# rafaelvp-db/databricks-distributed-deep-learning

Hardware: AMD Instinct MI355X
Metric: ResNet-50 images/sec (whole node) (higher is better)
Workload: dtype bf16

## Files before the change

csrc/kernels/norm.hip:

```cpp
#include "ddl_common.h"
#include <cstdlib>
#include <mutex>
#include <unordered_map>

namespace {

constexpr int BN_NT = 256;

template <typename T>
__global__ __launch_bounds__(BN_NT) void bn_stats_partial_k(const T* __restrict__ x, long M, int C,
                                                            int rows_per_blk, float* __restrict__ part) {
    __shared__ float s_red[2 * BN_NT * 8];
    const int tpr = C / 8;
    const int rpi = BN_NT / tpr;
    const int tid = threadIdx.x;
    const int cg = tid % tpr, rr = tid / tpr;
    const long r0 = (long)blockIdx.x * rows_per_blk;
    const long r1 = min(M, r0 + rows_per_blk);
    float s[8], q[8];
#pragma unroll
    for (int j = 0; j < 8; ++j) { s[j] = 0.f; q[j] = 0.f; }
    long r = r0 + rr;
    for (; r + 3 * rpi < r1; r += 4 * rpi) {
        float v[4][8];
// ... 352 lines not shown
                                                           const T* __restrict__ x, const float* __restrict__ mean,
                                                           const float* __restrict__ invstd,
                                                           const float* __restrict__ coef, T* __restrict__ dx,
                                                           T* __restrict__ dres, long M, int C) {
    const int tpr = C / 8, rpb = 256 / tpr;
    const int cg = threadIdx.x % tpr, rr = threadIdx.x / tpr;
    float A[8], B[8], D[8];
    {
        float mu[8], is[8], k1[8], mb[8], mg[8];
        load8(mean + cg * 8, mu);
        load8(invstd + cg * 8, is);
        load8(coef + cg * 8, k1);
        load8(coef + C + cg * 8, mb);
        load8(coef + 2 * C + cg * 8, mg);
#pragma unroll
        for (int j = 0; j < 8; ++j) {
            A[j] = k1[j];
            B[j] = -k1[j] * is[j] * mg[j];
            D[j] = k1[j] * (mu[j] * is[j] * mg[j] - mb[j]);
        }
    }
    const long rs = (long)gridDim.x * rpb;
    auto one = [&](const float* g, const float* xv, uint32_t bits, long row) {
        float o[8], dz[8];
#pragma unroll
        for (int j = 0; j < 8; ++j) {
            dz[j] = ((bits >> j) & 1u) ? g[j] : 0.f;
            o[j] = A[j] * dz[j] + B[j] * xv[j] + D[j];
        }
        store8(dx + row * C + cg * 8, o);
        if (DRES) store8(dres + row * C + cg * 8, dz);
    };
    long r = (long)blockIdx.x * rpb + rr;
    for (; r + 3 * rs < M; r += 4 * rs) {
        float g[4][8], xv[4][8];
        uint32_t bits[4];
#pragma unroll
        for (int u = 0; u < 4; ++u) {
            load8_nt(dy + (r + u * rs) * C + cg * 8, g[u]);
            load8_nt(x + (r + u * rs) * C + cg * 8, xv[u]);
            bits[u] = RELU ? mask[(r + u * rs) * tpr + cg] : 0xffu;
        }
#pragma unroll
        for (int u = 0; u < 4; ++u) one(g[u], xv[u], bits[u], r + u * rs);
    }
    for (; r < M; r += rs) {
        float g[8], xv[8];
        load8(dy + r * C + cg * 8, g);
        load8(x + r * C + cg * 8, xv);
        one(g, xv, RELU ? mask[r * tpr + cg] : 0xffu, r);
    }
}

template <typename T> struct Raw4;
template <> struct Raw4<bf16_t> { typedef uint2 type; };
template <> struct Raw4<float> { typedef float4 type; };
__device__ __forceinline__ uint2 ld_raw4(const bf16_t* p) { return *reinterpret_cast<const uint2*>(p); }
__device__ __forceinline__ float4 ld_raw4(const float* p) { return *reinterpret_cast<const float4*>(p); }
__device__ __forceinline__ void cvt_raw4(const uint2& u, float* v) {
    v[0] = __uint_as_float(u.x << 16); v[1] = __uint_as_float(u.x & 0xffff0000u);
    v[2] = __uint_as_float(u.y << 16); v[3] = __uint_as_float(u.y & 0xffff0000u);
}
__device__ __forceinline__ void cvt_raw4(const float4& a, float* v) { v[0] = a.x; v[1] = a.y; v[2] = a.z; v[3] = a.w; }

struct Drop {
    uint64_t seed;
    uint32_t thresh;
    float scale;
    void* dres;
};
__device__ __forceinline__ uint32_t drop_bits4(const Drop& d, long idx) {
    return keep_bits4(d.seed, (uint64_t)idx, d.thresh);
}
__device__ __forceinline__ void apply4(const Drop& d, uint32_t bits, float* v) {
#pragma unroll
    for (int j = 0; j < 4; ++j) v[j] = ((bits >> j) & 1u) ? v[j] * d.scale : 0.f;
}
__device__ __forceinline__ void drop4(const Drop& d, long idx, float* v) { apply4(d, drop_bits4(d, idx), v); }

template <typename T, int VPL>
__global__ __launch_bounds__(256) void ln_fwd_k(const T* __restrict__ x, const T* __restrict__ res, long res_rows,
                                                const T* __restrict__ gamma, const T* __restrict__ beta, T* __restrict__ y,
                                                float* __restrict__ save_mean, float* __restrict__ save_rstd, long rows,
                                                int H, float eps, Drop drop) {
    const int lane = threadIdx.x & 63;
    const long row = (long)blockIdx.x * 4 + (threadIdx.x >> 6);
    if (row >= rows) return;
    float v[VPL][4];
    float s = 0.f;
#pragma unroll
    for (int k = 0; k < VPL; ++k) {
        const int col = 256 * k + 4 * lane;
        load4(x + row * H + col, v[k]);
        if (drop.thresh) drop4(drop, row * H + col, v[k]);
        if (res) {
            float r[4];
            load4(res + (row % res_rows) * H + col, r);
#pragma unroll
            for (int j = 0; j < 4; ++j) v[k][j] += r[j];
        }
#pragma unroll
        for (int j = 0; j < 4; ++j) s += v[k][j];
    }
    const float mean = wave_sum_dpp(s) / H;
    float q = 0.f;
#pragma unroll
// ... 584 lines not shown
                                                                  eps, scale, shift);
    else
        bn_eval_coeffs_k<float><<<(C + 255) / 256, 256, 0, st>>>(C, (const float*)gamma, (const float*)beta, rm, rv,
                                                                 eps, scale, shift);
    DDL_RETURN_LAUNCH();
}

template <typename T>
static void bn_apply_dispatch(const T* x, const T* res, const float* sc, const float* sh, T* y, uint8_t* mask, long n,
                              int C, int relu, hipStream_t st) {
    if (rows_ok(C) && n % C == 0) {
        const long M = n / C;
        auto k = res ? (relu ? bn_apply_rows_k<T, true, true> : bn_apply_rows_k<T, true, false>)
                     : (relu ? bn_apply_rows_k<T, false, true> : bn_apply_rows_k<T, false, false>);
        hipLaunchKernelGGL(k, dim3(rows_grid(M, C, (const void*)k)), dim3(256), 0, st, x, res, sc, sh, y, mask, M, C);
        return;
    }
    const long n8 = n / 8;
    const int g = grid_for(n8, 256, 8192);
    if (res) {
        if (relu) bn_apply_k<T, true, true><<<g, 256, 0, st>>>(x, res, sc, sh, y, mask, n8, C);
        else bn_apply_k<T, true, false><<<g, 256, 0, st>>>(x, res, sc, sh, y, mask, n8, C);
    } else {
        if (relu) bn_apply_k<T, false, true><<<g, 256, 0, st>>>(x, res, sc, sh, y, mask, n8, C);
        else bn_apply_k<T, false, false><<<g, 256, 0, st>>>(x, res, sc, sh, y, mask, n8, C);
    }
}

DDL_API int ddl_bn_apply2(int dtype, const void* x, const void* x2, const float* scale, const float* shift,
                          const float* scale2, const float* shift2, void* y, long n, int C, int relu, void* mask,
                          hipStream_t st) {
    if (n % 8 || !rows_ok(C) || n % C) return -1;
    const long M = n / C;
    uint8_t* mk = (uint8_t*)mask;
#define BA2(T) do { auto k = relu ? bn_apply2_rows_k<T, true> : bn_apply2_rows_k<T, false>; \
                    hipLaunchKernelGGL(k, dim3(rows_grid(M, C, (const void*)k)), dim3(256), 0, st, (const T*)x, (const T*)x2, \
                                       scale, shift, scale2, shift2, (T*)y, mk, M, C); } while (0)
    if (dtype == 1) BA2(bf16_t);
    else BA2(float);
#undef BA2
    DDL_RETURN_LAUNCH();
}

DDL_API int ddl_bn_apply(int dtype, const void* x, const void* res, const float* scale, const float* shift, void* y,
                         long n, int C, int relu, void* mask, hipStream_t st) {
    if (n % 8 || C % 8) return -1;
    uint8_t* mk = (uint8_t*)mask;
    if (dtype == 1) bn_apply_dispatch((const bf16_t*)x, (const bf16_t*)res, scale, shift, (bf16_t*)y, mk, n, C, relu, st);
    else bn_apply_dispatch((const float*)x, (const float*)res, scale, shift, (float*)y, mk, n, C, relu, st);
    DDL_RETURN_LAUNCH();
}

template <typename T>
static void bwd_finalize(const float* part, int nblk, float* ws, int C, long M, const T* gamma, const float* invstd,
                         T* dgamma, T* dbeta, float* coef, int acc, hipStream_t st) {
    if (merged_finalize(nblk, C)) {
        const int S = fin_slices(nblk);
        int* tk = S > 1 ? fin_tickets() : nullptr;
        if (S == 1 || tk) {
            if (!ws) ws = const_cast<float*>(part) + (long)nblk * 2 * C;
            bn_bwd_finalize2_k<T><<<dim3((C + 63) / 64, S), 1024, 0, st>>>(part, nblk, fin_rps(nblk), C, M, ws, tk,
                                                                           gamma, invstd, dgamma, dbeta, coef, acc);
            return;
        }
    }
    int nrows = nblk;
    const float* fin = collapse_partials(part, nrows, 2 * C, st, ws);
    bn_bwd_finalize_k<T><<<(C + 63) / 64, 1024, 0, st>>>(fin, nrows, C, M, gamma, invstd, dgamma, dbeta, coef, acc);
}

template <typename T>
static void bn_bwd_dispatch(const T* dy, const uint8_t* yout, const T* x, const float* mean, const float* invstd,
                            const T* gamma, long M, int C, int relu, float* part, T* dgamma, T* dbeta, float* coef,
                            T* dx, T* dres, int acc, hipStream_t st) {
    const int nblk = ddl_bn_bwd_nblk(M, C);
    const int rpi = BN_NT / (C / 8);
    long rpb = (M + nblk - 1) / nblk;
    rpb = (rpb + rpi - 1) / rpi * rpi;
    if (relu) bn_bwd_partial_k<T, true><<<nblk, BN_NT, 0, st>>>(dy, yout, x, mean, invstd, M, C, (int)rpb, part);
    else bn_bwd_partial_k<T, false><<<nblk, BN_NT, 0, st>>>(dy, yout, x, mean, invstd, M, C, (int)rpb, part);
    bwd_finalize<T>(part, nblk, nullptr, C, M, gamma, invstd, dgamma, dbeta, coef, acc, st);
    if (rows_ok(C)) {
        auto k = relu ? (dres ? bn_bwd_apply_rows_k<T, true, true> : bn_bwd_apply_rows_k<T, true, false>)
                      : (dres ? bn_bwd_apply_rows_k<T, false, true> : bn_bwd_apply_rows_k<T, false, false>);
        hipLaunchKernelGGL(k, dim3(rows_grid(M, C, (const void*)k)), dim3(256), 0, st, dy, yout, x, mean, invstd, coef,
                           dx, dres, M, C);
        return;
    }
    const long n8 = M * C / 8;
    const int g = grid_for(n8, 256, 8192);
    if (relu) {
        if (dres) bn_bwd_apply_k<T, true, true><<<g, 256, 0, st>>>(dy, yout, x, mean, invstd, coef, dx, dres, n8, C);
        else bn_bwd_apply_k<T, true, false><<<g, 256, 0, st>>>(dy, yout, x, mean, invstd, coef, dx, dres, n8, C);
    } else {
        if (dres) bn_bwd_apply_k<T, false, true><<<g, 256, 0, st>>>(dy, yout, x, mean, invstd, coef, dx, dres, n8, C);
        else bn_bwd_apply_k<T, false, false><<<g, 256, 0, st>>>(dy, yout, x, mean, invstd, coef, dx, dres, n8, C);
    }
}

DDL_API int ddl_bn_bwd(int dtype, const void* dy, const void* mask, const void* x, const float* mean,
                       const float* invstd, const void* gamma, long M, int C, int relu, float* part, void* dgamma,
                       void* dbeta, float* coef, void* dx, void* dres, int acc_params, hipStream_t st) {
    if (C % 8 || (BN_NT % (C / 8) != 0) || (relu && !mask)) return -1;
    const uint8_t* yout = (const uint8_t*)mask;
    if (dtype == 1)
        bn_bwd_dispatch((const bf16_t*)dy, yout, (const bf16_t*)x, mean, invstd, (const bf16_t*)gamma, M,
                        C, relu, part, (bf16_t*)dgamma, (bf16_t*)dbeta, coef, (bf16_t*)dx, (bf16_t*)dres, acc_params, st);
    else
        bn_bwd_dispatch((const float*)dy, yout, (const float*)x, mean, invstd, (const float*)gamma, M, C,
                        relu, part, (float*)dgamma, (float*)dbeta, coef, (float*)dx, (float*)dres, acc_params, st);
    DDL_RETURN_LAUNCH();
}

namespace {
template <typename T>
__device__ __forceinline__ void pool_grad8(const T* __restrict__ dy, const uint8_t* __restrict__ idx, long n, int h,
                                           int w, int cg, int C, int P, int Q, float* acc) {
#pragma unroll
    for (int j = 0; j < 8; ++j) acc[j] = 0.f;
    const int p_lo = h >> 1, p_hi = min(P - 1, (h + 1) >> 1);
    const int q_lo = w >> 1, q_hi = min(Q - 1, (w + 1) >> 1);
    for (int p = p_lo; p <= p_hi; ++p) {
        const int r = h - 2 * p + 1;
        for (int q = q_lo; q <= q_hi; ++q) {
            const int s_ = w - 2 * q + 1;
            const long o = ((n * P + p) * Q + q) * C + cg * 8;
            float g[8];
            load8(dy + o, g);
            const uint2 packed = *reinterpret_cast<const uint2*>(idx + o);
            const uint32_t want = (uint32_t)(r * 3 + s_);
#pragma unroll
            for (int j = 0; j < 8; ++j) {
                const uint32_t word = j < 4 ? packed.x : packed.y;
                acc[j] += ((word >> (8 * (j & 3))) & 0xffu) == want ? g[j] : 0.f;
// ... 270 lines not shown
    __shared__ float red[1024];
    const int c = blockIdx.x * 64 + (threadIdx.x & 63);
    const float s = colsum64(part, nrows, width, c, c < n, red);
    if (threadIdx.x < 64 && c < n) sink[c] = from_f<TP>(s + (acc ? to_f(sink[c]) : 0.f));
}
}

DDL_API int ddl_rows_sum_sink(int dtype, const float* part, int nblk, int width, int n, void* sink, int acc,
                              float* ws, hipStream_t st) {
    if (n > width) return -1;
    int nrows = nblk;
    const float* src = collapse_partials(part, nrows, width, st, ws);
    if (dtype == 1) rows_sum_sink_k<bf16_t><<<(n + 63) / 64, 1024, 0, st>>>(src, nrows, width, n, (bf16_t*)sink, acc);
    else rows_sum_sink_k<float><<<(n + 63) / 64, 1024, 0, st>>>(src, nrows, width, n, (float*)sink, acc);
    DDL_RETURN_LAUNCH();
}

DDL_API int ddl_bn_rows_sum(const float* part, int nblk, int width, float* out, float* ws, hipStream_t st) {
    int nrows = nblk;
    const float* src = collapse_partials(part, nrows, width, st, ws);
    rows_sum_k<<<(width + 63) / 64, 1024, 0, st>>>(src, nrows, width, out);
    DDL_RETURN_LAUNCH();
}

DDL_API int ddl_bn_stats_partials(int dtype, const void* x, long M, int C, float* part, hipStream_t st) {
    if (C % 8 || (BN_NT % (C / 8) != 0)) return -1;
    const int nblk = ddl_bn_stats_nblk(M, C);
    const int rpi = BN_NT / (C / 8);
    long rpb = (M + nblk - 1) / nblk;
    rpb = (rpb + rpi - 1) / rpi * rpi;
    if (dtype == 1) bn_stats_partial_k<bf16_t><<<nblk, BN_NT, 0, st>>>((const bf16_t*)x, M, C, (int)rpb, part);
    else bn_stats_partial_k<float><<<nblk, BN_NT, 0, st>>>((const float*)x, M, C, (int)rpb, part);
    DDL_RETURN_LAUNCH();
}

DDL_API int ddl_bn_bwd_partials(int dtype, const void* dy, const void* mask, const void* x, const float* mean,
                                const float* invstd, long M, int C, int relu, float* part, hipStream_t st) {
    if (C % 8 || (BN_NT % (C / 8) != 0) || (relu && !mask)) return -1;
    const int nblk = ddl_bn_bwd_nblk(M, C);
    const int rpi = BN_NT / (C / 8);
    long rpb = (M + nblk - 1) / nblk;
    rpb = (rpb + rpi - 1) / rpi * rpi;
    const uint8_t* mk = (const uint8_t*)mask;
#define BWP(T) do { if (relu) bn_bwd_partial_k<T, true><<<nblk, BN_NT, 0, st>>>((const T*)dy, mk, (const T*)x, mean, invstd, M, C, (int)rpb, part); \
                    else bn_bwd_partial_k<T, false><<<nblk, BN_NT, 0, st>>>((const T*)dy, mk, (const T*)x, mean, invstd, M, C, (int)rpb, part); } while (0)
    if (dtype == 1) BWP(bf16_t);
    else BWP(float);
#undef BWP
    DDL_RETURN_LAUNCH();
}

template <typename T>
static void bn_bwd_apply_only(const T* dy, const uint8_t* mk, const T* x, const float* mean, const float* invstd,
                              long M, int C, int relu, const float* coef, T* dx, T* dres, hipStream_t st) {
    if (!rows_ok(C)) return;
    auto k = relu ? (dres ? bn_bwd_apply_rows_k<T, true, true> : bn_bwd_apply_rows_k<T, true, false>)
                  : (dres ? bn_bwd_apply_rows_k<T, false, true> : bn_bwd_apply_rows_k<T, false, false>);
    hipLaunchKernelGGL(k, dim3(rows_grid(M, C, (const void*)k)), dim3(256), 0, st, dy, mk, x, mean, invstd, coef, dx,
                       dres, M, C);
}

template <typename T>
static void bn_bwd_finish_t(const T* dy, const uint8_t* mk, const T* x, const float* mean, const float* invstd,
                            const T* gamma, long M, long M_total, int C, int relu, const float* row, int nrows,
                            T* dgamma, T* dbeta, float* coef, T* dx, T* dres, int acc, hipStream_t st,
                            const float* prow = nullptr) {
    bn_bwd_finalize_k<T><<<(C + 63) / 64, 1024, 0, st>>>(row, nrows, C, M_total, gamma, invstd, dgamma, dbeta, coef,
                                                         acc, prow);
    bn_bwd_apply_only(dy, mk, x, mean, invstd, M, C, relu, coef, dx, dres, st);
}

DDL_API int ddl_bn_bwd_finish(int dtype, const void* dy, const void* mask, const void* x, const float* mean,
                              const float* invstd, const void* gamma, long M, long M_total, int C, int relu,
                              const float* row, const float* local_row, void* dgamma, void* dbeta, float* coef,
                              void* dx, void* dres, int acc_params, hipStream_t st) {
    if (!rows_ok(C) || (relu && !mask)) return -1;
    const uint8_t* mk = (const uint8_t*)mask;
    if (dtype == 1)
        bn_bwd_finish_t((const bf16_t*)dy, mk, (const bf16_t*)x, mean, invstd, (const bf16_t*)gamma, M, M_total, C,
                        relu, row, 1, (bf16_t*)dgamma, (bf16_t*)dbeta, coef, (bf16_t*)dx, (bf16_t*)dres, acc_params, st,
                        local_row);
    else
        bn_bwd_finish_t((const float*)dy, mk, (const float*)x, mean, invstd, (const float*)gamma, M, M_total, C,
                        relu, row, 1, (float*)dgamma, (float*)dbeta, coef, (float*)dx, (float*)dres, acc_params, st,
                        local_row);
    DDL_RETURN_LAUNCH();
}

DDL_API int ddl_bn_bwd_from_partials(int dtype, const float* part, int nrows, float* ws, long ws_elems,
                                     const void* dz, const void* x, const float* mean, const float* invstd,
                                     const void* gamma, long M, int C, void* dgamma, void* dbeta, float* coef, void* dx,
                                     void* dres, int acc_params, hipStream_t st) {
    if (!rows_ok(C) || dtype != 1) return -1;
    if (merged_finalize(nrows, C) && (fin_slices(nrows) == 1 || (ws && ws_elems >= (long)fin_slices(nrows) * 2 * C))) {
        bwd_finalize<bf16_t>(part, nrows, fin_slices(nrows) == 1 ? nullptr : ws, C, M, (const bf16_t*)gamma, invstd,
                             (bf16_t*)dgamma, (bf16_t*)dbeta, coef, acc_params, st);
        bn_bwd_apply_only((const bf16_t*)dz, nullptr, (const bf16_t*)x, mean, invstd, M, C, 0, coef, (bf16_t*)dx,
                          (bf16_t*)dres, st);
        DDL_RETURN_LAUNCH();
    }
    const long need = ddl_bn_partials_ws(nrows, C);
    if (need > 0 && (!ws || ws_elems < need)) return -2;
    if (need > 0) {
        bwd_finalize<bf16_t>(part, nrows, ws, C, M, (const bf16_t*)gamma, invstd, (bf16_t*)dgamma, (bf16_t*)dbeta, coef,
                             acc_params, st);
        bn_bwd_apply_only((const bf16_t*)dz, nullptr, (const bf16_t*)x, mean, invstd, M, C, 0, coef, (bf16_t*)dx,
                          (bf16_t*)dres, st);
        DDL_RETURN_LAUNCH();
    }
    bn_bwd_finish_t((const bf16_t*)dz, nullptr, (const bf16_t*)x, mean, invstd, (const bf16_t*)gamma, M, M, C, 0, part,
                    nrows, (bf16_t*)dgamma, (bf16_t*)dbeta, coef, (bf16_t*)dx, (bf16_t*)dres, acc_params, st);
    DDL_RETURN_LAUNCH();
}
```

databricks_distributed_deep_learning_amd/ops/_lib.py:

```python
from __future__ import annotations

import ctypes
import os
from typing import Optional

import torch

_PKG_DIR = os.path.dirname(os.path.dirname(os.path.abspath(__file__)))
LIB_PATH = os.environ.get("DDL_NATIVE_LIB") or os.path.join(_PKG_DIR, "_native", "libddl_kernels.so")

_lib: Optional[ctypes.CDLL] = None
_load_error: Optional[str] = None
_mode = os.environ.get("DDL_NATIVE", "auto").lower()


class NativeUnavailable(RuntimeError):
    pass


def set_mode(mode: str) -> None:
    global _mode
    if mode not in ("auto", "on", "off"):
        raise ValueError(mode)
    _mode = mode
# ... 32 lines not shown


def available() -> bool:
    return load() is not None


def load_error() -> Optional[str]:
    load()
    return _load_error


def use_native(*tensors: torch.Tensor) -> bool:
    if _mode == "off":
        return False
    if not all(t is None or t.is_cuda for t in tensors):
        return False
    if load() is None:
        raise NativeUnavailable(
            f"HIP kernel library unavailable on a GPU run: {_load_error}. "
            "Build it with `python csrc/build.py` or set DDL_NATIVE=off for stock PyTorch ops.")
    return True


def get() -> ctypes.CDLL:
    lib = load()
    if lib is None:
        raise NativeUnavailable(_load_error)
    return lib


def stream() -> ctypes.c_void_p:
    return ctypes.c_void_p(torch.cuda.current_stream().cuda_stream)


def ptr(t: Optional[torch.Tensor]) -> ctypes.c_void_p:
    return ctypes.c_void_p(0 if t is None else t.data_ptr())


def check(rc: int, what: str) -> None:
    if rc != 0:
        raise RuntimeError(f"native kernel {what} failed with HIP error {rc}")


P, I, L, F, U64 = ctypes.c_void_p, ctypes.c_int, ctypes.c_long, ctypes.c_float, ctypes.c_uint64
_SIGS = {
    "ddl_bn_stats_nblk": [L, I],
    "ddl_bn_bwd_nblk": [L, I],
    "ddl_bn_rows_sum": [P, I, I, P, P, P],
    "ddl_rows_sum_sink": [I, P, I, I, I, P, I, P, P],
    "ddl_bn_stats_partials": [I, P, L, I, P, P],
    "ddl_bn_bwd_partials": [I, P, P, P, P, P, L, I, I, P, P],
    "ddl_bn_bwd_finish": [I, P, P, P, P, P, P, L, L, I, I, P, P, P, P, P, P, P, I, P],
    "ddl_bn_bwd_from_partials": [I, P, I, P, L, P, P, P, P, P, L, I, P, P, P, P, P, I, P],
    "ddl_bn_partials_ws": [I, I],
    "ddl_bn_fwd_train": [I, P, L, I, P, P, P, P, F, F, P, P, P, P, P, P],
    "ddl_bn_eval_coeffs": [I, I, P, P, P, P, F, P, P, P],
    "ddl_bn_apply": [I, P, P, P, P, P, L, I, I, P, P],
    "ddl_bn_apply2": [I, P, P, P, P, P, P, P, L, I, I, P, P],
    "ddl_bn_relu_maxpool": [I, P, P, P, P, P, P, I, I, I, I, I, I, P],
    "ddl_bn_bwd_pool_nblk": [],
    "ddl_bn_bwd_pool": [I, P, P, P, P, P, P, P, I, I, I, I, I, I, P, P, P, P, P, I, P],
    "ddl_bn_fwd_from_partials": [I, P, I, L, I, P, P, P, P, F, F, P, P, P, P, P, L],
    "ddl_conv_w_dgrad": [P, P, I, I, I, I, I, I, P, P, P],
    "ddl_conv_w_dgrad_batch": [P, P, I, P],
    "ddl_gelu_bwd_colsum": [I, P, P, P, L, I, P, P, I, I, P],
    "ddl_acc_f32": [I, P, P, L, P],
    "ddl_tanh_bwd": [I, P, P, P, L, P],
    "ddl_copy2d": [I, P, L, L, L, P, L, L, L, P],
    "ddl_add_into": [I, P, P, L, P],
    "ddl_zero": [P, L, P],
    "ddl_rows_add_row": [I, P, P, P, L, L, P],
    "ddl_seq_prepend_add": [I, P, P, P, P, L, L, L, P],
    "ddl_sort_ids_ok": [L, L],
    "ddl_sort_ids": [P, L, P, P, P],
    "ddl_drain_acc": [I, P, P, L, P],
    "ddl_acc_grad": [I, P, P, L, I, I, P],
    "ddl_softmax_topk": [I, P, L, I, I, P, P, P, P],
    "ddl_gemm_conv_multi": [I, I, P, P, P, P, P, L, I, P, P],
    "ddl_conv3x3": [P, P, P, I, I, I, I, I, P, P, P, P, P, P, I, P],
    "ddl_conv3x3_wgrad": [P, P, P, I, I, I, I, I, P, L, I, I, I, P],
    "ddl_stem_wgrad": [P, P, P, I, I, I, I, I, I, I, P, L, I, I, I, P],
    "ddl_stem_fwd": [P, P, P, I, I, I, I, P, I, P],
    "ddl_s2d_input": [P, I, I, I, I, I, P, I, I, P],
    "ddl_s2d_weight": [P, I, I, I, I, P, I, I, P],
    "ddl_skinny_gemm": [P, P, P, L, I, I, P, P, P, P, P, P, I, P],
    "ddl_stream_gemm": [P, P, P, L, I, I, P, P, P, P, P, P, I, P],
    "ddl_stream_wgrad_ws": [I, I],
    "ddl_bn_bwd": [I, P, P, P, P, P, P, L, I, I, P, P, P, P, P, P, I, P],
    "ddl_ln_supported": [I],
    "ddl_ln_fwd": [I, P, P, L, P, P, P, P, P, L, I, F, U64, F, P],
    "ddl_ln_bwd_nblk": [L],
    "ddl_ln_bwd": [I, P, P, P, L, P, P, P, P, P, P, P, L, I, I, P, U64, F, P, P, P, P],
    "ddl_gelu_fwd": [I, P, P, L, P],
    "ddl_gelu_bwd": [I, P, P, P, L, P],
    "ddl_dropout": [I, P, P, L, U64, F, P],
    "ddl_colsum_nblk": [L],
    "ddl_colsum": [I, P, L, I, P, P, I, I, P],
    "ddl_softmax_ce": [I, P, P, L, I, P, P, P, P],
    "ddl_scale_by": [I, P, P, P, L, P],
    "ddl_maxpool_fwd": [I, P, P, P, I, I, I, I, I, I, I, I, I, P],
    "ddl_maxpool_bwd": [I, P, P, P, I, I, I, I, I, I, I, I, I, P],
    "ddl_avgpool_fwd": [I, P, P, I, I, I, P],
    "ddl_avgpool_bwd": [I, P, P, I, I, I, P],
    "ddl_embedding_fwd": [I, P, P, P, L, I, P],
    "ddl_embedding_bwd": [I, P, P, P, P, L, L, I, I, P],
    "ddl_embedding_bwd_sorted": [I, P, P, P, P, P, L, I, I, P],
# ... 99 lines not shown
```

databricks_distributed_deep_learning_amd/ops/_native_norm.py:

```python
from __future__ import annotations

import os
from types import SimpleNamespace
from typing import Optional

import torch

from . import _lib
from ._native_elementwise import new_seed
from ._lib import call, dcode, grad_ready, grad_sink, p

_BN_BWD_EPI = os.environ.get("DDL_BN_BWD_EPI", "1") != "0"
_BN_BWD_EPI_RES = os.environ.get("DDL_BN_BWD_EPI", "1") not in ("0", "nores")


_LN_BIAS_SINK = os.environ.get("DDL_LN_BIAS_SINK", "1") != "0"


def _bn_supported(C: int) -> bool:
    return C % 8 == 0 and 256 % (C // 8) == 0


def _group_sum(row: torch.Tensor, group) -> None:
    import torch.distributed as dist
    from ..parallel import comm as _comm
    eng = _comm.active()
    if eng is not None and row.is_cuda and (group is None or group is dist.group.WORLD
                                            or dist.get_world_size(group) == eng.world):
        eng.wait_upto(eng.all_reduce(row))
        return
    dist.all_reduce(row, op=dist.ReduceOp.SUM, group=group)


def _bn_train_stats(x, weight, bias, running_mean, running_var, momentum, eps, given, stats) -> None:
    C = x.shape[-1]
    M = x.numel() // C
    dt = dcode(x)
    f32 = dict(dtype=torch.float32, device=x.device)
    if given is not None:
        part, nblk = given
        ws = torch.empty(-(-nblk // 32) * 2 * C, **f32) if nblk > 32 else None
        call("ddl_bn_fwd_from_partials", dt, p(part), nblk, M, C, p(weight), p(bias), p(running_mean),
             p(running_var), float(momentum), float(eps), p(stats[0]), p(stats[1]), p(stats[2]), p(stats[3]),
             p(ws), 0 if ws is None else ws.numel())
    else:
        nblk = _lib.fn("ddl_bn_stats_nblk")(M, C)
        part = torch.empty(nblk * 2 * C, **f32)
        call("ddl_bn_fwd_train", dt, p(x), M, C, p(weight), p(bias), p(running_mean), p(running_var),
             float(momentum), float(eps), p(part), p(stats[0]), p(stats[1]), p(stats[2]), p(stats[3]))


class _BatchNormTrain(torch.autograd.Function):
    @staticmethod
    def forward(ctx, x, weight, bias, running_mean, running_var, momentum, eps, relu, residual, bridge=None,
                pre=None, group=None):
        ctx.bridge = bridge
        ctx.group = group
        x = x.contiguous()
        C = x.shape[-1]
        M = x.numel() // C
        dt = dcode(x)
        f32 = dict(dtype=torch.float32, device=x.device)
        stats = torch.empty(4, C, **f32)
        given = pre.take_for(x) if pre is not None else None
        if group is not None:
            import torch.distributed as dist
            world = dist.get_world_size(group)
            if given is not None:
                part, nblk = given
                ws = torch.empty(-(-nblk // 32) * 2 * C, **f32)
            else:
                nblk = _lib.fn("ddl_bn_stats_nblk")(M, C)
                part = torch.empty((nblk + -(-nblk // 32)) * 2 * C, **f32)
                call("ddl_bn_stats_partials", dt, p(x), M, C, p(part))
                ws = None
            row = torch.empty(2 * C, **f32)
            call("ddl_bn_rows_sum", p(part), nblk, 2 * C, p(row), p(ws))
            _group_sum(row, group)
            call("ddl_bn_fwd_from_partials", dt, p(row), 1, M * world, C, p(weight), p(bias), p(running_mean),
                 p(running_var), float(momentum), float(eps), p(stats[0]), p(stats[1]), p(stats[2]), p(stats[3]),
                 None, 0)
            ctx.m_total = M * world
        else:
            _bn_train_stats(x, weight, bias, running_mean, running_var, momentum, eps, given, stats)
        res = residual.contiguous() if residual is not None else None
        y = torch.empty_like(x)
        mask = torch.empty(x.numel() // 8, dtype=torch.uint8, device=x.device) if relu else None
        call("ddl_bn_apply", dt, p(x), p(res), p(stats[2]), p(stats[3]), p(y), x.numel(), C, int(relu), p(mask))
        ctx.relu = bool(relu)
        ctx.has_res = residual is not None
        ctx.params = (weight, bias)
        ctx.save_for_backward(x, mask, weight, stats)
        ctx.bnb = None
        if _BN_BWD_EPI and x.dtype == torch.bfloat16:
            from .bridge import BNBackward
            ctx.bnb = BNBackward(x, mask, stats[0], stats[1])
            y._ddl_bnb = ctx.bnb
        return y

    @staticmethod
    def backward(ctx, dy):
        x, mask, weight, stats = ctx.saved_tensors
        dx, dgamma, dbeta, dres = _bn_backward(ctx, dy, x, mask, weight, stats)
        return dx, dgamma, dbeta, None, None, None, None, None, dres, None, None, None


def _bn_backward(ctx, dy, x, mask, weight, stats):
    dy = dy.contiguous()
    C = x.shape[-1]
    M = x.numel() // C
    nblk = _lib.fn("ddl_bn_bwd_nblk")(M, C)
    f32 = dict(dtype=torch.float32, device=x.device)
    part = torch.empty((nblk + -(-nblk // 32)) * 2 * C, **f32)
    coef = torch.empty(3 * C, **f32)
    dx = torch.empty_like(x)
    sg, sb = grad_sink(ctx.params[0]), grad_sink(ctx.params[1])
    direct = sg is not None and sb is not None
    if direct:
        dgamma, dbeta = sg, sb
    else:
        dgamma = torch.empty_like(weight) if weight is not None else None
        dbeta = torch.empty_like(weight) if weight is not None else None
    given = ctx.bnb.take_for(dy) if ctx.bnb is not None else None
    ctx.bnb = None
    dres = torch.empty_like(x) if ctx.has_res and (given is None or ctx.group is not None) else None
    if given is not None:
        gpart, nrows = given
        if ctx.group is not None:
            row = torch.empty(2 * C, **f32)
            call("ddl_bn_rows_sum", p(gpart), nrows, 2 * C, p(row), None)
            local = row.clone()
            _group_sum(row, ctx.group)
            call("ddl_bn_bwd_finish", dcode(x), p(dy), None, p(x), p(stats[0]), p(stats[1]), p(weight), M,
                 ctx.m_total, C, 0, p(row), p(local), p(dgamma), p(dbeta), p(coef), p(dx), p(dres), int(direct))
        else:
            ws = gpart[nrows * 2 * C:]
            call("ddl_bn_bwd_from_partials", dcode(x), p(gpart), nrows, p(ws), ws.numel(), p(dy), p(x),
                 p(stats[0]), p(stats[1]), p(weight), M, C, p(dgamma), p(dbeta), p(coef), p(dx), None,
                 int(direct))
            if ctx.has_res:
                dres = dy
    elif ctx.group is not None:
        call("ddl_bn_bwd_partials", dcode(x), p(dy), p(mask), p(x), p(stats[0]), p(stats[1]), M, C,
             int(ctx.relu), p(part))
        row = torch.empty(2 * C, **f32)
        call("ddl_bn_rows_sum", p(part), nblk, 2 * C, p(row), None)
        local = row.clone()
        _group_sum(row, ctx.group)
        call("ddl_bn_bwd_finish", dcode(x), p(dy), p(mask), p(x), p(stats[0]), p(stats[1]), p(weight), M,
             ctx.m_total, C, int(ctx.relu), p(row), p(local), p(dgamma), p(dbeta), p(coef), p(dx), p(dres),
             int(direct))
    else:
        call("ddl_bn_bwd", dcode(x), p(dy), p(mask), p(x), p(stats[0]), p(stats[1]), p(weight), M, C,
             int(ctx.relu), p(part), p(dgamma), p(dbeta), p(coef), p(dx), p(dres), int(direct))
    if direct:
        grad_ready(ctx.params[0])
        grad_ready(ctx.params[1])
        dgamma = dbeta = None
    if dres is not None and ctx.bridge is not None:
        ctx.bridge.put(dres)
        dres = None
    return dx, dgamma, dbeta, dres


class _BatchNormAddBNTrain(torch.autograd.Function):

    @staticmethod
    def forward(ctx, x, weight, bias, running_mean, running_var, momentum, eps, x2, weight2, bias2, running_mean2,
                running_var2, momentum2, eps2, pre=None, pre2=None):
        x, x2 = x.contiguous(), x2.contiguous()
        C = x.shape[-1]
        f32 = dict(dtype=torch.float32, device=x.device)
        stats = torch.empty(4, C, **f32)
        stats2 = torch.empty(4, C, **f32)
        _bn_train_stats(x, weight, bias, running_mean, running_var, momentum, eps,
                        pre.take_for(x) if pre is not None else None, stats)
        _bn_train_stats(x2, weight2, bias2, running_mean2, running_var2, momentum2, eps2,
                        pre2.take_for(x2) if pre2 is not None else None, stats2)
        y = torch.empty_like(x)
        mask = torch.empty(x.numel() // 8, dtype=torch.uint8, device=x.device)
        call("ddl_bn_apply2", dcode(x), p(x), p(x2), p(stats[2]), p(stats[3]), p(stats2[2]), p(stats2[3]), p(y),
             x.numel(), C, 1, p(mask))
        ctx.bridge, ctx.group, ctx.relu, ctx.has_res = None, None, True, True
        ctx.params, ctx.params2 = (weight, bias), (weight2, bias2)
        ctx.save_for_backward(x, mask, weight, stats, x2, weight2, stats2)
        ctx.bnb = None
        if _BN_BWD_EPI and x.dtype == torch.bfloat16:
            from .bridge import BNBackward
            ctx.bnb = BNBackward(x, mask, stats[0], stats[1])
            y._ddl_bnb = ctx.bnb
        return y

    @staticmethod
    def backward(ctx, dy):
        x, mask, weight, stats, x2, weight2, stats2 = ctx.saved_tensors
        dx, dgamma, dbeta, dres = _bn_backward(ctx, dy, x, mask, weight, stats)
        c2 = SimpleNamespace(bnb=None, group=None, has_res=False, relu=False, params=ctx.params2, bridge=None)
        dx2, dgamma2, dbeta2, _ = _bn_backward(c2, dres, x2, None, weight2, stats2)
        return (dx, dgamma, dbeta, None, None, None, None, dx2, dgamma2, dbeta2, None, None, None, None, None, None)


class _BNReluMaxPoolTrain(torch.autograd.Function):

    @staticmethod
    def forward(ctx, x, weight, bias, running_mean, running_var, momentum, eps, pre=None):
        x = x.contiguous()
        N, H, W, C = x.shape
        P, Q = H // 2, W // 2
        stats = torch.empty(4, C, dtype=torch.float32, device=x.device)
        _bn_train_stats(x, weight, bias, running_mean, running_var, momentum, eps,
                        pre.take_for(x) if pre is not None else None, stats)
        y = torch.empty(N, P, Q, C, dtype=x.dtype, device=x.device)
        idx = torch.empty(N, P, Q, C, dtype=torch.uint8, device=x.device)
        mask = torch.empty(x.numel() // 8, dtype=torch.uint8, device=x.device)
        call("ddl_bn_relu_maxpool", dcode(x), p(x), p(stats[2]), p(stats[3]), p(y), p(idx), p(mask), N, H, W, C, P, Q)
        ctx.params = (weight, bias)
        ctx.save_for_backward(x, mask, weight, stats, idx)
        return y

    @staticmethod
    def backward(ctx, dy):
        x, mask, weight, stats, idx = ctx.saved_tensors
        N, H, W, C = x.shape
        dy = dy.contiguous()
        if not _FUSED_STEM_BWD:
            da = torch.empty_like(x)
            call("ddl_maxpool_bwd", dcode(dy), p(dy), p(idx), p(da), N, H, W, C, H // 2, W // 2, 3, 2, 1)
            c = SimpleNamespace(bnb=None, group=None, has_res=False, relu=True, params=ctx.params, bridge=None)
            dx, dgamma, dbeta, _ = _bn_backward(c, da, x, mask, weight, stats)
            return dx, dgamma, dbeta, None, None, None, None, None
        nblk = _lib.fn("ddl_bn_bwd_pool_nblk")()
        f32 = dict(dtype=torch.float32, device=x.device)
        part = torch.empty((nblk + -(-nblk // 32)) * 2 * C, **f32)
        coef = torch.empty(3 * C, **f32)
        dx = torch.empty_like(x)
        sg, sb = grad_sink(ctx.params[0]), grad_sink(ctx.params[1])
        direct = sg is not None and sb is not None
        dgamma, dbeta = (sg, sb) if direct else (torch.empty_like(weight), torch.empty_like(weight))
        call("ddl_bn_bwd_pool", dcode(x), p(dy), p(idx), p(mask), p(x), p(stats[0]), p(stats[1]), p(weight), N, H, W,
             C, H // 2, W // 2, p(part), p(dgamma), p(dbeta), p(coef), p(dx), int(direct))
        if direct:
            grad_ready(ctx.params[0])
            grad_ready(ctx.params[1])
            dgamma = dbeta = None
        return dx, dgamma, dbeta, None, None, None, None, None


def bn_relu_maxpool(x, weight, bias, running_mean, running_var, momentum, eps, pre=None):
    N, H, W, C = x.shape
    if (not _FUSED_STEM or not _bn_supported(C) or x.dtype not in (torch.bfloat16, torch.float32)
# ... 170 lines not shown
```

Measured before the change: 12700.

## Fuse second BN's backward partial reduction into first BN's backward apply kernel

In the dual-BN residual block backward, the first BN's apply kernel now also reads x2 and accumulates the second BN's per-channel partial sums (dz times normalized x2) into part2. The second BN backward then consumes these partials through the existing BNBackward bridge. This removes a separate partial-stats pass over dres and x2. In exchange the apply kernel does extra loads and register work, and it needs a shared-memory reduction per block.

```diff
diff --git a/csrc/kernels/norm.hip b/csrc/kernels/norm.hip
--- a/csrc/kernels/norm.hip
+++ b/csrc/kernels/norm.hip
@@ -428,6 +428,81 @@
     }
 }
 
+template <typename T, bool RELU, bool DRES>
+__global__ __launch_bounds__(256) void bn_bwd_apply_ride_k(const T* __restrict__ dy, const uint8_t* __restrict__ mask,
+                                                           const T* __restrict__ x, const float* __restrict__ mean,
+                                                           const float* __restrict__ invstd,
+                                                           const float* __restrict__ coef, T* __restrict__ dx,
+                                                           T* __restrict__ dres, long M, int C,
+                                                           const T* __restrict__ x2, const float* __restrict__ mean2,
+                                                           const float* __restrict__ invstd2,
+                                                           float* __restrict__ part2) {
+    __shared__ float s_red[256 * 8];
+    const int tpr = C / 8, rpb = 256 / tpr;
+    const int cg = threadIdx.x % tpr, rr = threadIdx.x / tpr;
+    float A[8], B[8], D[8], mu2[8], is2[8], q[8];
+    {
+        float mu[8], is[8], k1[8], mb[8], mg[8];
+        load8(mean + cg * 8, mu);
+        load8(invstd + cg * 8, is);
+        load8(coef + cg * 8, k1);
+        load8(coef + C + cg * 8, mb);
+        load8(coef + 2 * C + cg * 8, mg);
+#pragma unroll
+        for (int j = 0; j < 8; ++j) {
+            A[j] = k1[j];
+            B[j] = -k1[j] * is[j] * mg[j];
+            D[j] = k1[j] * (mu[j] * is[j] * mg[j] - mb[j]);
+            q[j] = 0.f;
+        }
+        load8(mean2 + cg * 8, mu2);
+        load8(invstd2 + cg * 8, is2);
+    }
+    const long rs = (long)gridDim.x * rpb;
+    auto one = [&](const float* g, const float* xv, const float* x2v, uint32_t bits, long row) {
+        float o[8], dz[8];
+#pragma unroll
+        for (int j = 0; j < 8; ++j) {
+            dz[j] = ((bits >> j) & 1u) ? g[j] : 0.f;
+            o[j] = A[j] * dz[j] + B[j] * xv[j] + D[j];
+            q[j] += dz[j] * (x2v[j] - mu2[j]) * is2[j];
+        }
+        store8(dx + row * C + cg * 8, o);
+        if (DRES) store8(dres + row * C + cg * 8, dz);
+    };
+    long r = (long)blockIdx.x * rpb + rr;
+    for (; r + rs < M; r += 2 * rs) {
+        float g[2][8], xv[2][8], x2v[2][8];
+        uint32_t bits[2];
+#pragma unroll
+        for (int u = 0; u < 2; ++u) {
+            load8(dy + (r + u * rs) * C + cg * 8, g[u]);
+            load8_nt(x + (r + u * rs) * C + cg * 8, xv[u]);
+            load8(x2 + (r + u * rs) * C + cg * 8, x2v[u]);
+            bits[u] = RELU ? mask[(r + u * rs) * tpr + cg] : 0xffu;
+        }
+#pragma unroll
+        for (int u = 0; u < 2; ++u) one(g[u], xv[u], x2v[u], bits[u], r + u * rs);
+    }
+    for (; r < M; r += rs) {
+        float g[8], xv[8], x2v[8];
+        load8(dy + r * C + cg * 8, g);
+        load8(x + r * C + cg * 8, xv);
+        load8(x2 + r * C + cg * 8, x2v);
+        one(g, xv, x2v, RELU ? mask[r * tpr + cg] : 0xffu, r);
+    }
+#pragma unroll
+    for (int j = 0; j < 8; ++j) s_red[threadIdx.x * 8 + j] = q[j];
+    __syncthreads();
+    float* row = part2 + (long)blockIdx.x * 2 * C;
+    for (int c = threadIdx.x; c < C; c += 256) {
+        float s = 0.f;
+        for (int i = 0; i < rpb; ++i) s += s_red[i * C + c];
+        row[c] = blockIdx.x == 0 ? coef[C + c] * (float)M : 0.f;
+        row[C + c] = s;
+    }
+}
+
 template <typename T> struct Raw4;
 template <> struct Raw4<bf16_t> { typedef uint2 type; };
 template <> struct Raw4<float> { typedef float4 type; };
@@ -1118,6 +1193,27 @@
 }
 
 template <typename T>
+struct Ride {
+    const T* x2;
+    const float *mean2, *invstd2;
+    float* part2;
+    int nblk2;
+};
+template <typename T>
+static auto ride_kernel(int relu, bool dres) {
+    return relu ? (dres ? bn_bwd_apply_ride_k<T, true, true> : bn_bwd_apply_ride_k<T, true, false>)
+                : (dres ? bn_bwd_apply_ride_k<T, false, true> : bn_bwd_apply_ride_k<T, false, false>);
+}
+template <typename T>
+static void bn_bwd_apply_ride(const T* dy, const uint8_t* mk, const T* x, const float* mean, const float* invstd,
+                              long M, int C, int relu, const float* coef, T* dx, T* dres, const Ride<T>& rd,
+                              hipStream_t st) {
+    auto k = ride_kernel<T>(relu, dres != nullptr);
+    hipLaunchKernelGGL(k, dim3(rd.nblk2), dim3(256), 0, st, dy, mk, x, mean, invstd, coef, dx,
+                       dres, M, C, rd.x2, rd.mean2, rd.invstd2, rd.part2);
+}
+
+template <typename T>
 static void bwd_finalize(const float* part, int nblk, float* ws, int C, long M, const T* gamma, const float* invstd,
                          T* dgamma, T* dbeta, float* coef, int acc, hipStream_t st) {
     if (merged_finalize(nblk, C)) {
@@ -1138,7 +1234,7 @@
 template <typename T>
 static void bn_bwd_dispatch(const T* dy, const uint8_t* yout, const T* x, const float* mean, const float* invstd,
                             const T* gamma, long M, int C, int relu, float* part, T* dgamma, T* dbeta, float* coef,
-                            T* dx, T* dres, int acc, hipStream_t st) {
+                            T* dx, T* dres, int acc, hipStream_t st, const Ride<T>* ride = nullptr) {
     const int nblk = ddl_bn_bwd_nblk(M, C);
     const int rpi = BN_NT / (C / 8);
     long rpb = (M + nblk - 1) / nblk;
@@ -1146,6 +1242,10 @@
     if (relu) bn_bwd_partial_k<T, true><<<nblk, BN_NT, 0, st>>>(dy, yout, x, mean, invstd, M, C, (int)rpb, part);
     else bn_bwd_partial_k<T, false><<<nblk, BN_NT, 0, st>>>(dy, yout, x, mean, invstd, M, C, (int)rpb, part);
     bwd_finalize<T>(part, nblk, nullptr, C, M, gamma, invstd, dgamma, dbeta, coef, acc, st);
+    if (ride) {
+        bn_bwd_apply_ride(dy, yout, x, mean, invstd, M, C, relu, coef, dx, dres, *ride, st);
+        return;
+    }
     if (rows_ok(C)) {
         auto k = relu ? (dres ? bn_bwd_apply_rows_k<T, true, true> : bn_bwd_apply_rows_k<T, true, false>)
                       : (dres ? bn_bwd_apply_rows_k<T, false, true> : bn_bwd_apply_rows_k<T, false, false>);
@@ -1522,8 +1622,13 @@
 
 template <typename T>
 static void bn_bwd_apply_only(const T* dy, const uint8_t* mk, const T* x, const float* mean, const float* invstd,
-                              long M, int C, int relu, const float* coef, T* dx, T* dres, hipStream_t st) {
+                              long M, int C, int relu, const float* coef, T* dx, T* dres, hipStream_t st,
+                              const Ride<T>* ride = nullptr) {
     if (!rows_ok(C)) return;
+    if (ride) {
+        bn_bwd_apply_ride(dy, mk, x, mean, invstd, M, C, relu, coef, dx, dres, *ride, st);
+        return;
+    }
     auto k = relu ? (dres ? bn_bwd_apply_rows_k<T, true, true> : bn_bwd_apply_rows_k<T, true, false>)
                   : (dres ? bn_bwd_apply_rows_k<T, false, true> : bn_bwd_apply_rows_k<T, false, false>);
     hipLaunchKernelGGL(k, dim3(rows_grid(M, C, (const void*)k)), dim3(256), 0, st, dy, mk, x, mean, invstd, coef, dx,
@@ -1534,10 +1639,10 @@
 static void bn_bwd_finish_t(const T* dy, const uint8_t* mk, const T* x, const float* mean, const float* invstd,
                             const T* gamma, long M, long M_total, int C, int relu, const float* row, int nrows,
                             T* dgamma, T* dbeta, float* coef, T* dx, T* dres, int acc, hipStream_t st,
-                            const float* prow = nullptr) {
+                            const float* prow = nullptr, const Ride<T>* ride = nullptr) {
     bn_bwd_finalize_k<T><<<(C + 63) / 64, 1024, 0, st>>>(row, nrows, C, M_total, gamma, invstd, dgamma, dbeta, coef,
                                                          acc, prow);
-    bn_bwd_apply_only(dy, mk, x, mean, invstd, M, C, relu, coef, dx, dres, st);
+    bn_bwd_apply_only(dy, mk, x, mean, invstd, M, C, relu, coef, dx, dres, st, ride);
 }
 
 DDL_API int ddl_bn_bwd_finish(int dtype, const void* dy, const void* mask, const void* x, const float* mean,
@@ -1557,16 +1662,16 @@
     DDL_RETURN_LAUNCH();
 }
 
-DDL_API int ddl_bn_bwd_from_partials(int dtype, const float* part, int nrows, float* ws, long ws_elems,
-                                     const void* dz, const void* x, const float* mean, const float* invstd,
-                                     const void* gamma, long M, int C, void* dgamma, void* dbeta, float* coef, void* dx,
-                                     void* dres, int acc_params, hipStream_t st) {
+static int bn_bwd_from_partials(int dtype, const float* part, int nrows, float* ws, long ws_elems, const void* dz,
+                                const void* x, const float* mean, const float* invstd, const void* gamma, long M,
+                                int C, void* dgamma, void* dbeta, float* coef, void* dx, void* dres, int acc_params,
+                                hipStream_t st, const Ride<bf16_t>* ride = nullptr) {
     if (!rows_ok(C) || dtype != 1) return -1;
     if (merged_finalize(nrows, C) && (fin_slices(nrows) == 1 || (ws && ws_elems >= (long)fin_slices(nrows) * 2 * C))) {
         bwd_finalize<bf16_t>(part, nrows, fin_slices(nrows) == 1 ? nullptr : ws, C, M, (const bf16_t*)gamma, invstd,
                              (bf16_t*)dgamma, (bf16_t*)dbeta, coef, acc_params, st);
         bn_bwd_apply_only((const bf16_t*)dz, nullptr, (const bf16_t*)x, mean, invstd, M, C, 0, coef, (bf16_t*)dx,
-                          (bf16_t*)dres, st);
+                          (bf16_t*)dres, st, ride);
         DDL_RETURN_LAUNCH();
     }
     const long need = ddl_bn_partials_ws(nrows, C);
@@ -1575,10 +1680,46 @@
         bwd_finalize<bf16_t>(part, nrows, ws, C, M, (const bf16_t*)gamma, invstd, (bf16_t*)dgamma, (bf16_t*)dbeta, coef,
                              acc_params, st);
         bn_bwd_apply_only((const bf16_t*)dz, nullptr, (const bf16_t*)x, mean, invstd, M, C, 0, coef, (bf16_t*)dx,
-                          (bf16_t*)dres, st);
+                          (bf16_t*)dres, st, ride);
         DDL_RETURN_LAUNCH();
     }
     bn_bwd_finish_t((const bf16_t*)dz, nullptr, (const bf16_t*)x, mean, invstd, (const bf16_t*)gamma, M, M, C, 0, part,
-                    nrows, (bf16_t*)dgamma, (bf16_t*)dbeta, coef, (bf16_t*)dx, (bf16_t*)dres, acc_params, st);
+                    nrows, (bf16_t*)dgamma, (bf16_t*)dbeta, coef, (bf16_t*)dx, (bf16_t*)dres, acc_params, st, nullptr,
+                    ride);
     DDL_RETURN_LAUNCH();
 }
+
+DDL_API int ddl_bn_bwd_from_partials(int dtype, const float* part, int nrows, float* ws, long ws_elems,
+                                     const void* dz, const void* x, const float* mean, const float* invstd,
+                                     const void* gamma, long M, int C, void* dgamma, void* dbeta, float* coef, void* dx,
+                                     void* dres, int acc_params, hipStream_t st) {
+    return bn_bwd_from_partials(dtype, part, nrows, ws, ws_elems, dz, x, mean, invstd, gamma, M, C, dgamma, dbeta, coef,
+                                dx, dres, acc_params, st);
+}
+
+DDL_API int ddl_bn_bwd_ride_nblk(long M, int C, int relu, int dres) {
+    if (!rows_ok(C)) return -1;
+    return rows_grid(M, C, (const void*)ride_kernel<bf16_t>(relu, dres != 0));
+}
+
+DDL_API int ddl_bn_bwd_from_partials_ride(int dtype, const float* part, int nrows, float* ws, long ws_elems,
+                                          const void* dz, const void* x, const float* mean, const float* invstd,
+                                          const void* gamma, long M, int C, void* dgamma, void* dbeta, float* coef,
+                                          void* dx, int acc_params, const void* x2, const float* mean2,
+                                          const float* invstd2, float* part2, int nblk2, hipStream_t st) {
+    if (!rows_ok(C) || dtype != 1 || !x2 || !part2 || nblk2 < 1) return -1;
+    const Ride<bf16_t> rd{(const bf16_t*)x2, mean2, invstd2, part2, nblk2};
+    return bn_bwd_from_partials(dtype, part, nrows, ws, ws_elems, dz, x, mean, invstd, gamma, M, C, dgamma, dbeta, coef,
+                                dx, nullptr, acc_params, st, &rd);
+}
+
+DDL_API int ddl_bn_bwd_ride(int dtype, const void* dy, const void* mask, const void* x, const float* mean,
+                            const float* invstd, const void* gamma, long M, int C, int relu, float* part, void* dgamma,
+                            void* dbeta, float* coef, void* dx, void* dres, int acc_params, const void* x2,
+                            const float* mean2, const float* invstd2, float* part2, int nblk2, hipStream_t st) {
+    if (!rows_ok(C) || BN_NT % (C / 8) != 0 || dtype != 1 || (relu && !mask) || !x2 || !part2 || nblk2 < 1) return -1;
+    const Ride<bf16_t> rd{(const bf16_t*)x2, mean2, invstd2, part2, nblk2};
+    bn_bwd_dispatch((const bf16_t*)dy, (const uint8_t*)mask, (const bf16_t*)x, mean, invstd, (const bf16_t*)gamma, M, C,
+                    relu, part, (bf16_t*)dgamma, (bf16_t*)dbeta, coef, (bf16_t*)dx, (bf16_t*)dres, acc_params, st, &rd);
+    DDL_RETURN_LAUNCH();
+}
diff --git a/databricks_distributed_deep_learning_amd/ops/_lib.py b/databricks_distributed_deep_learning_amd/ops/_lib.py
--- a/databricks_distributed_deep_learning_amd/ops/_lib.py
+++ b/databricks_distributed_deep_learning_amd/ops/_lib.py
@@ -108,6 +108,9 @@
     "ddl_bn_bwd_partials": [I, P, P, P, P, P, L, I, I, P, P],
     "ddl_bn_bwd_finish": [I, P, P, P, P, P, P, L, L, I, I, P, P, P, P, P, P, P, I, P],
     "ddl_bn_bwd_from_partials": [I, P, I, P, L, P, P, P, P, P, L, I, P, P, P, P, P, I, P],
+    "ddl_bn_bwd_ride_nblk": [L, I, I, I],
+    "ddl_bn_bwd_from_partials_ride": [I, P, I, P, L, P, P, P, P, P, L, I, P, P, P, P, I, P, P, P, P, I, P],
+    "ddl_bn_bwd_ride": [I, P, P, P, P, P, P, L, I, I, P, P, P, P, P, P, I, P, P, P, P, I, P],
     "ddl_bn_partials_ws": [I, I],
     "ddl_bn_fwd_train": [I, P, L, I, P, P, P, P, F, F, P, P, P, P, P, P],
     "ddl_bn_eval_coeffs": [I, I, P, P, P, P, F, P, P, P],
diff --git a/databricks_distributed_deep_learning_amd/ops/_native_norm.py b/databricks_distributed_deep_learning_amd/ops/_native_norm.py
--- a/databricks_distributed_deep_learning_amd/ops/_native_norm.py
+++ b/databricks_distributed_deep_learning_amd/ops/_native_norm.py
@@ -12,6 +12,7 @@
 
 _BN_BWD_EPI = os.environ.get("DDL_BN_BWD_EPI", "1") != "0"
 _BN_BWD_EPI_RES = os.environ.get("DDL_BN_BWD_EPI", "1") not in ("0", "nores")
+_BN_BWD_RIDE = os.environ.get("DDL_BN_BWD_EPI", "1") == "1"
 
 
 _LN_BIAS_SINK = os.environ.get("DDL_LN_BIAS_SINK", "1") != "0"
@@ -105,7 +106,7 @@
         return dx, dgamma, dbeta, None, None, None, None, None, dres, None, None, None
 
 
-def _bn_backward(ctx, dy, x, mask, weight, stats):
+def _bn_backward(ctx, dy, x, mask, weight, stats, ride=None):
     dy = dy.contiguous()
     C = x.shape[-1]
     M = x.numel() // C
@@ -124,6 +125,10 @@
     given = ctx.bnb.take_for(dy) if ctx.bnb is not None else None
     ctx.bnb = None
     dres = torch.empty_like(x) if ctx.has_res and (given is None or ctx.group is not None) else None
+    part2 = None
+    if ride is not None and ctx.group is None and ctx.has_res and x.dtype == torch.bfloat16:
+        nblk2 = _lib.fn("ddl_bn_bwd_ride_nblk")(M, C, int(ctx.relu and given is None), int(dres is not None))
+        part2 = torch.empty((nblk2 + -(-nblk2 // 32)) * 2 * C, **f32)
     if given is not None:
         gpart, nrows = given
         if ctx.group is not None:
@@ -135,9 +140,14 @@
                  ctx.m_total, C, 0, p(row), p(local), p(dgamma), p(dbeta), p(coef), p(dx), p(dres), int(direct))
         else:
             ws = gpart[nrows * 2 * C:]
-            call("ddl_bn_bwd_from_partials", dcode(x), p(gpart), nrows, p(ws), ws.numel(), p(dy), p(x),
-                 p(stats[0]), p(stats[1]), p(weight), M, C, p(dgamma), p(dbeta), p(coef), p(dx), None,
-                 int(direct))
+            if part2 is not None:
+                call("ddl_bn_bwd_from_partials_ride", dcode(x), p(gpart), nrows, p(ws), ws.numel(), p(dy), p(x),
+                     p(stats[0]), p(stats[1]), p(weight), M, C, p(dgamma), p(dbeta), p(coef), p(dx), int(direct),
+                     p(ride.x), p(ride.mean), p(ride.istd), p(part2), nblk2)
+            else:
+                call("ddl_bn_bwd_from_partials", dcode(x), p(gpart), nrows, p(ws), ws.numel(), p(dy), p(x),
+                     p(stats[0]), p(stats[1]), p(weight), M, C, p(dgamma), p(dbeta), p(coef), p(dx), None,
+                     int(direct))
             if ctx.has_res:
                 dres = dy
     elif ctx.group is not None:
@@ -150,9 +160,15 @@
         call("ddl_bn_bwd_finish", dcode(x), p(dy), p(mask), p(x), p(stats[0]), p(stats[1]), p(weight), M,
              ctx.m_total, C, int(ctx.relu), p(row), p(local), p(dgamma), p(dbeta), p(coef), p(dx), p(dres),
              int(direct))
+    elif part2 is not None:
+        call("ddl_bn_bwd_ride", dcode(x), p(dy), p(mask), p(x), p(stats[0]), p(stats[1]), p(weight), M, C,
+             int(ctx.relu), p(part), p(dgamma), p(dbeta), p(coef), p(dx), p(dres), int(direct),
+             p(ride.x), p(ride.mean), p(ride.istd), p(part2), nblk2)
     else:
         call("ddl_bn_bwd", dcode(x), p(dy), p(mask), p(x), p(stats[0]), p(stats[1]), p(weight), M, C,
              int(ctx.relu), p(part), p(dgamma), p(dbeta), p(coef), p(dx), p(dres), int(direct))
+    if part2 is not None:
+        ride.set(dres, part2, nblk2)
     if direct:
         grad_ready(ctx.params[0])
         grad_ready(ctx.params[1])
@@ -194,8 +210,12 @@
     @staticmethod
     def backward(ctx, dy):
         x, mask, weight, stats, x2, weight2, stats2 = ctx.saved_tensors
-        dx, dgamma, dbeta, dres = _bn_backward(ctx, dy, x, mask, weight, stats)
-        c2 = SimpleNamespace(bnb=None, group=None, has_res=False, relu=False, params=ctx.params2, bridge=None)
+        ride = None
+        if _BN_BWD_RIDE and x.dtype == torch.bfloat16:
+            from .bridge import BNBackward
+            ride = BNBackward(x2, None, stats2[0], stats2[1])
+        dx, dgamma, dbeta, dres = _bn_backward(ctx, dy, x, mask, weight, stats, ride)
+        c2 = SimpleNamespace(bnb=ride, group=None, has_res=False, relu=False, params=ctx.params2, bridge=None)
         dx2, dgamma2, dbeta2, _ = _bn_backward(c2, dres, x2, None, weight2, stats2)
         return (dx, dgamma, dbeta, None, None, None, None, dx2, dgamma2, dbeta2, None, None, None, None, None, None)
 
```

Result: no change. 12730, median of 6 (+0.2%).
